# aosokin/os2d

Measured on AMD Instinct MI355X. Metric: query-image-pairs/s (1280-px input, ResNet50, N-class), higher is better.
Workload: dtype fftx3 (as fft; the per-bin complex GEMM on the fp16 MFMA with spectra split into fp16 hi+lo, 3 MFMAs per product, fp32 accumulate)

## Files before the change

os2d_amd/csrc/dft_mfma.h:

```cpp
#pragma once

#ifndef DFT_DEV
#error "the includer defines DFT_DEV, DFT_TID, DFT_BID, DFT_GRID, DFT_LDS, DFT_BARRIER, DFT_MFMA, DFT_SHFL_XOR, DFT_SHFL_XOR_U32, DFT_BALLOT, DFT_FLAG, DFT_FLAG_SET, DFT_RAISE, DFT_UNIFORM"
#endif

#ifndef DFT_HD
#define DFT_HD static inline
#endif
#ifndef DFT_MEMBER
#define DFT_MEMBER inline
#endif
#ifndef DFT_LANDED
#define DFT_LANDED(X)
#endif
#ifndef DFT_FWD_PREFETCH_AFTER
#define DFT_FWD_PREFETCH_AFTER 2
#endif
#ifndef DFT_INV_PREFETCH_AFTER
#define DFT_INV_PREFETCH_AFTER 2
#endif
#ifndef DFT_PIPE_REGA
#define DFT_PIPE_REGA 1
#endif
#ifndef DFT_PIPE_LDS
#define DFT_PIPE_LDS 1
#endif
#ifndef DFT_SCHED_FENCE
#define DFT_SCHED_FENCE()
#endif
#ifndef DFT_STREAM_STORE
#define DFT_STREAM_STORE(P, V) (*(P) = (V))
#endif
#ifndef DFT_STAMP
#define DFT_STAMP(K)
#define DFT_STAMP_BEGIN()
#define DFT_STAMP_END(BASE)
#endif

#include "tile_common.h"

namespace os2d_dft {

typedef float f32x4u __attribute__((ext_vector_type(4), aligned(4)));

constexpr int DFT_THR = 512, DFT_WAVES = 8;
constexpr int DFT_G = 4;
constexpr int DFT_MAXP = 64;
constexpr int DFT_MAXV = 48;
constexpr int DFT_MAXWK = 96;
constexpr int DFT_KREG = 8;

struct DftPlan {
  int H, W;
  int P, Q, V, NBINS;
  int T, TY, TX, TH, TW;
  int oy, ox;
  int LH, LW;
  int RH;
  int Pp;
  int Wk;
  int N1;
  int M2;
  int Mx;
  int N2;
  int MA;
  int MB;
  int KB;
  int NBo;
  int G;
  int eT;
  int fast;
  unsigned inv_cg, inv_t, inv_tx, inv_c4, inv_v, inv_pq, inv_og, inv_kg, inv_pp;
  int lds_const, lds_union, lds_total;
};

DFT_HD int dft_round_up(int x, int m) { return (x + m - 1) / m * m; }
DFT_HD unsigned dft_magic(unsigned d) { return d > 1 ? (unsigned)(((1ull << 32) + d - 1) / d) : 0u; }

DFT_HD int dft_units_fqt(int P, int Q) { return (dft_round_up(Q, 16) / 8) * 2 * dft_round_up(Q + 2, 32); }
DFT_HD int dft_units_fp2(int P, int Q) { return (2 * dft_round_up(P, 8) / 8) * 2 * dft_round_up(2 * P, 32); }
DFT_HD int dft_units_e2(int P, int Q) { return (2 * dft_round_up(P, 8) / 8) * 2 * dft_round_up(2 * P, 32); }
DFT_HD int dft_units_gq(int P, int Q) { return (dft_round_up(Q + 2, 16) / 8) * 2 * dft_round_up(Q, 32); }
DFT_HD size_t dft_matrices_units(int P, int Q) {
  return (size_t)dft_units_fqt(P, Q) + dft_units_fp2(P, Q) + dft_units_e2(P, Q) + dft_units_gq(P, Q);
}

static inline bool dft_plan_transform(int LH, int LW, int RH, int ncols, int minP, int minQ, int G, DftPlan* pl) {
  pl->G = G;
  pl->P = dft_round_up(minP, 4);
  pl->Q = dft_round_up(minQ, 2);
  pl->V = pl->Q / 2 + 1;
  pl->NBINS = dft_round_up(pl->P * pl->V, 8);
  pl->LH = LH;
  pl->LW = LW;
  pl->RH = RH;
  pl->Pp = dft_round_up(pl->P, 8);
  pl->Wk = dft_round_up(LW, 16);
  pl->N1 = dft_round_up(2 * pl->V, 32);
  pl->M2 = dft_round_up(2 * pl->P, 32);
  pl->Mx = dft_round_up(G * pl->Pp, 32);
  pl->N2 = dft_round_up(G * pl->V, 32);
  pl->MA = dft_round_up(2 * RH, 32);
  pl->MB = G * (pl->MA / 2);
  pl->KB = dft_round_up(2 * pl->V, 16);
  pl->NBo = dft_round_up(ncols, 32);
  int e = 0;
  while ((1 << e) < pl->P) ++e;
  pl->eT = e + 1;
  if (pl->P > DFT_MAXP || pl->V > DFT_MAXV || pl->Wk > DFT_MAXWK || LH > pl->P || LW > pl->Q || RH > pl->P) return false;
  const int fqt = (pl->Wk / 8) * 2 * pl->N1 * 16, gq = (pl->KB / 8) * 2 * pl->NBo * 16;
  const int x = (pl->Wk / 8) * 2 * (pl->Mx + 1) * 16, r2 = (2 * pl->Pp / 8) * 2 * (pl->N2 + 1) * 16;
  const int xs = pl->V * (pl->P * 8 * G + 16);
  const int y2 = r2, tt = (pl->KB / 8) * 2 * (pl->MB + 1) * 16;
  int u = x;
  if (r2 > u) u = r2;
  if (xs > u) u = xs;
  if (y2 > u) u = y2;
  if (tt > u) u = tt;
  if (G == 8) {
    const int fp2 = (2 * pl->Pp / 8) * 2 * pl->M2 * 16;
    const int ca = fqt + fp2, cb = gq + fp2;
    pl->lds_const = ca > cb ? ca : cb;
    pl->lds_union = dft_round_up(u, 256);
    pl->lds_total = pl->lds_const + pl->lds_union + 1024;
    const int t1 = (pl->Mx / 32) * (pl->N1 / 32), t2 = (pl->M2 / 32) * (pl->N2 / 32), tA = (pl->MA / 32) * (pl->N2 / 32),
              tB = (pl->MB / 32) * (pl->NBo / 32);
    const int npos = pl->Pp * (pl->Wk / 4), nitem = G * pl->V * (pl->Pp / 8);
    return pl->lds_total <= 160 * 1024 && t1 <= 24 && t2 <= 24 && tA <= 24 && tB <= 24 && npos <= 2 * DFT_THR && nitem <= 3 * DFT_THR;
  }
  pl->lds_const = fqt > gq ? fqt : gq;
  pl->lds_union = dft_round_up(u, 256);
  pl->lds_total = pl->lds_const + pl->lds_union + 1024;
  return pl->lds_total <= 160 * 1024;
}

static inline void dft_set_tiles(DftPlan* pl, int H, int W, int TY, int TX, int TH, int TW) {
  pl->H = H;
  pl->W = W;
  pl->TY = TY;
  pl->TX = TX;
  pl->T = TY * TX;
  pl->TH = TH;
  pl->TW = TW;
  pl->oy = TY > 1 ? 3 : 0;
  pl->ox = TX > 1 ? 3 : 0;
  pl->fast = (pl->T == 1 && (W & 3) == 0) ? 1 : 0;
  pl->inv_t = dft_magic((unsigned)pl->T);
  pl->inv_tx = dft_magic((unsigned)TX);
  pl->inv_c4 = dft_magic((unsigned)(pl->Wk / 4));
  pl->inv_v = dft_magic((unsigned)pl->V);
  pl->inv_pq = dft_magic((unsigned)(pl->P / 4 * pl->G * 2));
  pl->inv_kg = dft_magic((unsigned)(pl->Pp / 8));
  pl->inv_pp = dft_magic((unsigned)pl->Pp);
}

struct DftSize {
  int P, Q;
};
static const DftSize DFT_CANONICAL[6] = {{36, 46}, {44, 54}, {48, 62}, {52, 68}, {56, 70}, {64, 84}};

static inline bool dft_make_plan_policy(int H, int W, int canonical, DftPlan* out, int G = DFT_G) {
  bool found = false;
  long best = 0;
  for (int TY = 1; TY <= 48; ++TY)
    for (int TX = 1; TX <= 48; ++TX) {
      const int TH = (H + TY - 1) / TY, TW = (W + TX - 1) / TX;
      if ((TY > 1 && (TY - 1) * TH >= H) || (TX > 1 && (TX - 1) * TW >= W)) continue;
      const int LH = TY > 1 ? TH + 6 : H, LW = TX > 1 ? TW + 6 : W;
      const int minP = TY > 1 ? TH + 6 : H + 3, minQ = TX > 1 ? TW + 6 : W + 3;
      if (minP > DFT_MAXP || minQ > 2 * (DFT_MAXV - 1)) continue;
      for (int k = 0; k < (canonical ? 6 : 1); ++k) {
        if (canonical && (DFT_CANONICAL[k].P < minP || DFT_CANONICAL[k].Q < minQ)) continue;
        DftPlan c = {};
        if (!dft_plan_transform(LH, LW, TY > 1 ? TH + 3 : H, TX > 1 ? TW + 3 : W, canonical ? DFT_CANONICAL[k].P : minP,
                                canonical ? DFT_CANONICAL[k].Q : minQ, G, &c))
          continue;
        dft_set_tiles(&c, H, W, TY, TX, TH, TW);
        const long cost = (long)c.T * c.NBINS;
        if (!found || cost < best) {
          found = true;
          best = cost;
          *out = c;
        }
      }
    }
  return found;
}

#ifndef OS2D_HOST_EMU
static inline int dft_size_policy() {
  static const int policy = [] {
    const char* e = getenv("OS2D_DFT_SIZES");
    return (e && (e[0] == 'e' || e[0] == '0')) ? 0 : 1;
  }();
  return policy;
}
#else
static inline int dft_size_policy() { return emu_dft_policy; }
#endif
static inline bool dft_make_plan(int H, int W, DftPlan* out) { return dft_make_plan_policy(H, W, dft_size_policy(), out); }
static inline bool dft_plan_g8(const DftPlan& base, DftPlan* out) {
  DftPlan c = {};
  if (!dft_plan_transform(base.LH, base.LW, base.RH, base.TX > 1 ? base.TW + 3 : base.W, base.P, base.Q, 8, &c)) return false;
  dft_set_tiles(&c, base.H, base.W, base.TY, base.TX, base.TH, base.TW);
  *out = c;
  return true;
}

constexpr int DFT_PBLK = 64;
DFT_HD size_t dft_spectra_pair0(int pr, int NBT, int NQ, int cstride, size_t* qstride) {
  const int pb = pr / DFT_PBLK, pl = pr - pb * DFT_PBLK;
  const int nbl = NBT - pb * DFT_PBLK < DFT_PBLK ? NBT - pb * DFT_PBLK : DFT_PBLK;
  *qstride = (size_t)nbl * cstride * 8;
  return ((size_t)pb * DFT_PBLK * NQ + pl) * cstride * 8;
}

DFT_DEV int dft_div(int x, unsigned magic) { return magic ? (int)(((unsigned long long)(unsigned)x * magic) >> 32) : x; }

DFT_DEV void dft_split4(float a, float b, float c, float d, u32x2* hi, u32x2* lo) {
  const f32x4 x = {a, b, c, d};
  const half4 h = __builtin_convertvector(x, half4);
  *hi = __builtin_bit_cast(u32x2, h);
#ifdef DFT_SPLIT_LO_PAIR
  u32x2 l;
  l[0] = DFT_SPLIT_LO_PAIR(a, b, (*hi)[0]);
  l[1] = DFT_SPLIT_LO_PAIR(c, d, (*hi)[1]);
  *lo = l;
#else
  const half4 l = __builtin_convertvector(x - __builtin_convertvector(h, f32x4), half4);
  *lo = __builtin_bit_cast(u32x2, l);
#endif
}

DFT_DEV half8 dft_frag(const u32x4* p) { return __builtin_bit_cast(half8, *p); }

DFT_DEV f32x16 dft_mma3(half8 ah, half8 al, half8 bh, half8 bl, f32x16 acc) {
  acc = DFT_MFMA(ah, bl, acc);
  acc = DFT_MFMA(al, bh, acc);
  acc = DFT_MFMA(ah, bh, acc);
  return acc;
}

template <int NT, int KS>
DFT_DEV void dft_product_rega(f32x16* acc, const half8* ah, const half8* al, int ksn, const u32x4* B, int bstride, int nt0,
                              int ntstep, int l31, int hw) {
  constexpr int KR = KS ? KS : DFT_KREG;
  half8 bh[2][NT], bl[2][NT];
#define DFT_REGA_READ(KSTEP, SET)                                                                                          \
  _Pragma("unroll") for (int j = 0; j < NT; ++j) {                                                                         \
    bh[SET][j] = dft_frag(B + (size_t)((2 * (KSTEP) + hw) * 2 + 0) * bstride + (nt0 + ntstep * j) * 32 + l31);             \
    bl[SET][j] = dft_frag(B + (size_t)((2 * (KSTEP) + hw) * 2 + 1) * bstride + (nt0 + ntstep * j) * 32 + l31);             \
  }
  if (DFT_PIPE_REGA) DFT_REGA_READ(0, 0)
#pragma unroll
  for (int ks = 0; ks < KR; ++ks) {
    if (KS || ks < ksn) {
      if (DFT_PIPE_REGA) {
        if (ks + 1 < KR && (KS || ks + 1 < ksn)) DFT_REGA_READ(ks + 1, (ks + 1) & 1)
        DFT_SCHED_FENCE();
      } else {
        DFT_REGA_READ(ks, ks & 1)
      }
#pragma unroll
      for (int j = 0; j < NT; ++j) acc[j] = dft_mma3(ah[ks], al[ks], bh[ks & 1][j], bl[ks & 1][j], acc[j]);
      if (DFT_PIPE_REGA) DFT_SCHED_FENCE();
    }
  }
#undef DFT_REGA_READ
}

template <int KS>
DFT_DEV void dft_product_rega_any(f32x16* acc, int ntiles, const half8* ah, const half8* al, int ksn, const u32x4* B, int bstride,
                                  int nt0, int ntstep, int l31, int hw) {
  if (ntiles == 3) dft_product_rega<3, KS>(acc, ah, al, ksn, B, bstride, nt0, ntstep, l31, hw);
  else if (ntiles == 2) dft_product_rega<2, KS>(acc, ah, al, ksn, B, bstride, nt0, ntstep, l31, hw);
  else if (ntiles == 1) dft_product_rega<1, KS>(acc, ah, al, ksn, B, bstride, nt0, ntstep, l31, hw);
}

template <int NT, bool SHARE, int NW, int PIPE_MODE>
DFT_DEV void dft_product_lds(f32x16* acc, int ks0, int ks1, const u32x4* A, int astride, const u32x4* B, int bstride, int t0, int mtn,
                             int l31, int hw) {
  constexpr int NA = SHARE ? 1 : NT;
  int tm[NT], tn[NT];
#pragma unroll
  for (int j = 0; j < NT; ++j) {
    const int t = t0 + NW * j;
    tn[j] = t / mtn;
    tm[j] = t - tn[j] * mtn;
  }
  half8 ah[2][NA], al[2][NA], bh[2][NT], bl[2][NT];
#define DFT_LDS_READ(KSTEP, SET)                                                                                           \
  {                                                                                                                        \
    const int kc_ = (KSTEP) < ks1 ? (KSTEP) : ks1 - 1;                                                                     \
    _Pragma("unroll") for (int j = 0; j < NA; ++j) {                                                                       \
      ah[SET][j] = dft_frag(A + (size_t)((2 * kc_ + hw) * 2 + 0) * astride + tm[j] * 32 + l31);                            \
      al[SET][j] = dft_frag(A + (size_t)((2 * kc_ + hw) * 2 + 1) * astride + tm[j] * 32 + l31);                            \
    }                                                                                                                      \
    _Pragma("unroll") for (int j = 0; j < NT; ++j) {                                                                       \
      bh[SET][j] = dft_frag(B + (size_t)((2 * kc_ + hw) * 2 + 0) * bstride + tn[j] * 32 + l31);                            \
      bl[SET][j] = dft_frag(B + (size_t)((2 * kc_ + hw) * 2 + 1) * bstride + tn[j] * 32 + l31);                            \
    }                                                                                                                      \
  }
#define DFT_LDS_MMA(SET)                                                                                                   \
  DFT_SCHED_FENCE();                                                                                                       \
  _Pragma("unroll") for (int j = 0; j < NT; ++j)                                                                           \
    acc[j] = dft_mma3(ah[SET][SHARE ? 0 : j], al[SET][SHARE ? 0 : j], bh[SET][j], bl[SET][j], acc[j]);                    \
  DFT_SCHED_FENCE();
  if (ks0 >= ks1) return;
  constexpr bool PIPE = PIPE_MODE == 2 || (PIPE_MODE == 1 && SHARE);
  if (!PIPE) {
    for (int ks = ks0; ks < ks1; ++ks) {
      DFT_LDS_READ(ks, 0)
      _Pragma("unroll") for (int j = 0; j < NT; ++j)
        acc[j] = dft_mma3(ah[0][SHARE ? 0 : j], al[0][SHARE ? 0 : j], bh[0][j], bl[0][j], acc[j]);
    }
    return;
  }
  DFT_LDS_READ(ks0, 0)
  int ks = ks0;
  for (; ks + 1 < ks1; ks += 2) {
    DFT_LDS_READ(ks + 1, 1)
    DFT_LDS_MMA(0)
    DFT_LDS_READ(ks + 2, 0)
    DFT_LDS_MMA(1)
  }
  if (ks < ks1) {
    DFT_LDS_MMA(0)
  }
#undef DFT_LDS_READ
#undef DFT_LDS_MMA
}

template <int NW, int PIPE_MODE>
DFT_DEV void dft_product_lds_any(f32x16* acc, int ntiles, int ks0, int ks1, const u32x4* A, int astride, const u32x4* B, int bstride,
                                 int t0, int mtn, int l31, int hw) {
  const bool share = mtn == NW;
  if (ntiles == 3) {
    if (share) dft_product_lds<3, true, NW, PIPE_MODE>(acc, ks0, ks1, A, astride, B, bstride, t0, mtn, l31, hw);
    else dft_product_lds<3, false, NW, PIPE_MODE>(acc, ks0, ks1, A, astride, B, bstride, t0, mtn, l31, hw);
  } else if (ntiles == 2) {
    if (share) dft_product_lds<2, true, NW, PIPE_MODE>(acc, ks0, ks1, A, astride, B, bstride, t0, mtn, l31, hw);
    else dft_product_lds<2, false, NW, PIPE_MODE>(acc, ks0, ks1, A, astride, B, bstride, t0, mtn, l31, hw);
  } else if (ntiles == 1) {
    dft_product_lds<1, true, NW, PIPE_MODE>(acc, ks0, ks1, A, astride, B, bstride, t0, mtn, l31, hw);
  }
}

DFT_DEV void dft_matrix_unit(int which, int unit, int P, int Q, const double* twP, const double* twQ, u32x4* out) {
  const int V = Q / 2 + 1, Pp = dft_round_up(P, 8);
  int cols, kidx, hl, col;
  double vals[8];
  if (which == 0) cols = dft_round_up(2 * V, 32);
  else if (which == 1 || which == 2) cols = dft_round_up(2 * P, 32);
  else cols = dft_round_up(Q, 32);
  col = unit % cols;
  hl = (unit / cols) & 1;
  kidx = unit / (2 * cols);
  for (int t = 0; t < 8; ++t) {
    const int k = kidx * 8 + t;
    double x = 0.0;
    if (which == 0) {
      const int v = col >> 1, ri = col & 1;
      if (k < Q && v < V) x = twQ[2 * (int)(((long long)v * k) % Q) + ri] * 16384.0;
    } else if (which == 1) {
      const int ri = k / Pp, h = k - ri * Pp, u = col >> 1, ro = col & 1;
      if (h < P && u < P && ri < 2) {
        const int a = (int)(((long long)u * h) % P);
        const double c = twP[2 * a], s = -twP[2 * a + 1];
        x = (ro == 0 ? (ri == 0 ? c : s) : (ri == 0 ? -s : c)) * 16384.0;
      }
    } else if (which == 2) {
      const int ri = k / Pp, u = k - ri * Pp, h = col >> 1, ro = col & 1;
      if (u < P && h < P && ri < 2) {
        const int a = (int)(((long long)u * h) % P);
        const double c = twP[2 * a], s = -twP[2 * a + 1];
        x = (ro == 0 ? (ri == 0 ? c : -s) : (ri == 0 ? s : c)) * 16384.0;
      }
    } else {
      const int v = k >> 1, ri = k & 1;
      if (v < V && col < Q) {
        const double a = (v == 0 || 2 * v == Q) ? 1.0 : 2.0;
        x = a * twQ[2 * (int)(((long long)v * col) % Q) + ri] * 8192.0;
      }
    }
    vals[t] = x;
  }
  unsigned w[4];
  for (int t = 0; t < 4; ++t) {
    unsigned short b[2];
    for (int e = 0; e < 2; ++e) {
      const double x = vals[2 * t + e];
      const _Float16 h = (_Float16)x;
      const _Float16 r = hl == 0 ? h : (_Float16)(x - (double)h);
      b[e] = __builtin_bit_cast(unsigned short, r);
    }
    w[t] = (unsigned)b[0] | ((unsigned)b[1] << 16);
  }
  u32x4 o;
  o[0] = w[0];
  o[1] = w[1];
  o[2] = w[2];
  o[3] = w[3];
  *out = o;
}

template <bool TILED, bool FAST, int G, int NW, int KS2 = 0>
DFT_DEV void dft_forward_body(const float* corr,
                              const float* invn,
                              float* X,
                              const u32x4* FqT, const u32x4* Fp2, const DftPlan& pl, int C, int Cpad, int NBT, int iters) {
  constexpr int THR = NW * 64;
  constexpr bool ALDS = G == 8;
  unsigned char* smem = DFT_LDS;
  const int tid = DFT_TID, lane = tid & 63, l31 = lane & 31, hw = lane >> 5;
  const int wv = DFT_UNIFORM(tid >> 6);
  const int P = pl.P, V = pl.V, Pp = pl.Pp, Wk = pl.Wk, N1 = pl.N1, Mx = pl.Mx, N2 = pl.N2, LH = pl.LH, LW = pl.LW, W = pl.W, H = pl.H;
  const int MxS = Mx + 1, N2S = N2 + 1;
  const int CG = (C + G - 1) / G, HW = H * W;
  u32x4* ldsF = reinterpret_cast<u32x4*>(smem);
  u32x4* ldsU = reinterpret_cast<u32x4*>(smem + pl.lds_const);
  unsigned char* ldsUb = smem + pl.lds_const;
  const int nF = (Wk / 8) * 2 * N1;
  for (int i = tid; i < nF; i += THR) ldsF[i] = FqT[i];
  u32x4* ldsP = ldsF + nF;
  if (ALDS)
    for (int i = tid; i < (2 * Pp / 8) * 2 * pl.M2; i += THR) ldsP[i] = Fp2[i];

  const int mt1n = Mx / 32, nt1n = N1 / 32, nt2n = N2 / 32, mt2n = pl.M2 / 32;
  const int ks1n = Wk / 16, ks2n = 2 * Pp / 16;
  const int mt2 = wv & 3;
  constexpr int KR2 = KS2 ? KS2 : DFT_KREG;
  half8 fp2h[KR2], fp2l[KR2];
  if (!ALDS) {
#pragma unroll
    for (int ks = 0; ks < KR2; ++ks) {
      const int kc = ks < ks2n ? ks : 0, mc = mt2 < mt2n ? mt2 : 0;
      fp2h[ks] = dft_frag(Fp2 + ((size_t)((2 * kc + hw) * 2 + 0)) * pl.M2 + mc * 32 + l31);
      fp2l[ks] = dft_frag(Fp2 + ((size_t)((2 * kc + hw) * 2 + 1)) * pl.M2 + mc * 32 + l31);
    }
  }
  if (!ALDS) {
#pragma unroll
    for (int ks = 0; ks < KR2; ++ks) {
      DFT_LANDED(fp2h[ks]);
      DFT_LANDED(fp2l[ks]);
    }
  }

  constexpr int NSLOT = ALDS ? 2 : 3 * 512 / THR;
  const int npos = Pp * (Wk / 4);
  f32x4 pc[NSLOT][G], pn[NSLOT];
#define DFT_FWD_ITER(IT)                                                                                     \
  const int pr_ = dft_div((IT), pl.inv_cg), cg_ = (IT)-pr_ * CG;                                             \
  const int nb_ = TILED ? dft_div(pr_, pl.inv_t) : pr_, tile_ = TILED ? pr_ - nb_ * pl.T : 0;               \
  const int ty_ = TILED ? dft_div(tile_, pl.inv_tx) : 0, tx_ = TILED ? tile_ - ty_ * pl.TX : 0;             \
  const int Y0 = TILED ? ty_ * pl.TH - pl.oy : 0, X0 = TILED ? tx_ * pl.TW - pl.ox : 0;                     \
  const int c0_ = cg_ * G;
#define DFT_FWD_POS(TID, S)                                                                                  \
  const int i_ = (TID) + (S)*THR;                                                                        \
  const int r_ = dft_div(i_, pl.inv_c4), c4_ = i_ - r_ * (Wk / 4);                                          \
  const int y_ = Y0 + r_, x_ = X0 + 4 * c4_;
#define DFT_FWD_PREFETCH(IT, TID) DFT_FWD_PREFETCH_SLOTS(IT, TID, 0, NSLOT)
#define DFT_FWD_PREFETCH_SLOTS(IT, TID, S0, S1)                                                              \
  {                                                                                                          \
    DFT_FWD_ITER(IT)                                                                                         \
    _Pragma("unroll") for (int s = (S0); s < (S1); ++s) {                                                    \
      DFT_FWD_POS(TID, s)                                                                                    \
      if (FAST) {                                                                                            \
        const bool ok = i_ < npos && r_ < LH && 4 * c4_ < LW;                                                \
        const int off = ok ? y_ * W + x_ : 0;                                                                \
        pn[s] = *reinterpret_cast<const f32x4*>(invn + (size_t)nb_ * HW + off);                             \
        _Pragma("unroll") for (int g = 0; g < G; ++g) {                                                  \
          const int c = c0_ + g < C ? c0_ + g : C - 1;                                                       \
          pc[s][g] = *reinterpret_cast<const f32x4*>(corr + ((size_t)nb_ * C + c) * HW + off);              \
        }                                                                                                    \
      } else {                                                                                               \
                                                                           \
        const bool rok = i_ < npos && r_ < LH && y_ >= 0 && y_ < H;                                          \
        const int off0 = y_ * W + x_;                                                                        \
        const bool vec = rok && off0 >= 0 && off0 + 3 < HW;                                                  \
        const int offv = vec ? off0 : 0;                                                                     \
        pn[s] = *reinterpret_cast<const f32x4u*>(invn + (size_t)nb_ * HW + offv);                            \
        _Pragma("unroll") for (int g = 0; g < G; ++g) {                                                      \
          const int c = c0_ + g < C ? c0_ + g : C - 1;                                                       \
          pc[s][g] = *reinterpret_cast<const f32x4u*>(corr + ((size_t)nb_ * C + c) * HW + offv);             \
        }                                                                                                    \
        if (rok && !vec) {                                                                                   \
          _Pragma("unroll") for (int e = 0; e < 4; ++e) {                                                    \
            const bool ok = 4 * c4_ + e < LW && x_ + e >= 0 && x_ + e < W;                                   \
            const int off = ok ? y_ * W + x_ + e : 0;                                                        \
            pn[s][e] = invn[(size_t)nb_ * HW + off];                                                         \
            _Pragma("unroll") for (int g = 0; g < G; ++g) {                                                  \
              const int c = c0_ + g < C ? c0_ + g : C - 1;                                                   \
              pc[s][g][e] = corr[((size_t)nb_ * C + c) * HW + off];                                          \
            }                                                                                                \
          }                                                                                                  \
        }                                                                                                    \
      }                                                                                                      \
    }                                                                                                        \
  }
  const int first = (DFT_GRID & 7) == 0 ? (DFT_BID & 7) * (DFT_GRID >> 3) + (DFT_BID >> 3) : DFT_BID;
  if (first < iters) DFT_FWD_PREFETCH(first, tid)
  DFT_BARRIER();

  DFT_STAMP_BEGIN()
  for (int it = first; it < iters; it += DFT_GRID) {
    int tl = tid;
#ifndef OS2D_HOST_EMU
    asm volatile("" : "+v"(tl));
#endif
    const int lane = tl & 63, l31 = lane & 31, hw = lane >> 5;
    DFT_FWD_ITER(it)
    {
#pragma unroll
      for (int s = 0; s < NSLOT; ++s) {
        DFT_FWD_POS(tl, s)
        if (i_ < npos) {
          float nsc[4];
#pragma unroll
          for (int e = 0; e < 4; ++e) {
            const bool ok = FAST ? (r_ < LH && 4 * c4_ < LW) : (r_ < LH && y_ >= 0 && y_ < H && 4 * c4_ + e < LW && x_ + e >= 0 && x_ + e < W);
            nsc[e] = ok ? pn[s][e] * 32768.0f : 0.f;
          }
#pragma unroll
          for (int g = 0; g < G; ++g) {
            u32x2 hi = {0u, 0u}, lo = {0u, 0u};
            if (c0_ + g < C)
              dft_split4(fmaxf(pc[s][g][0], 0.f) * nsc[0], fmaxf(pc[s][g][1], 0.f) * nsc[1], fmaxf(pc[s][g][2], 0.f) * nsc[2],
                         fmaxf(pc[s][g][3], 0.f) * nsc[3], &hi, &lo);
            const int m = g * Pp + r_;
            unsigned char* dst = ldsUb + ((size_t)((c4_ >> 1) * 2) * MxS + m) * 16 + (c4_ & 1) * 8;
            *reinterpret_cast<u32x2*>(dst) = hi;
            *reinterpret_cast<u32x2*>(dst + (size_t)MxS * 16) = lo;
          }
        }
      }
      for (int i = tid; i < (Mx - G * Pp) * (Wk / 8) * 2; i += THR) {
        const int m = G * Pp + i % (Mx - G * Pp), kh = i / (Mx - G * Pp);
        ldsU[(size_t)kh * MxS + m] = u32x4{0u, 0u, 0u, 0u};
      }
    }
    DFT_BARRIER();
    DFT_STAMP(0)

    f32x16 acc[3];
    int tm[3], tn[3];
    int nt1w = 0;
#pragma unroll
    for (int j = 0; j < 3; ++j) {
      const int t = wv + NW * j;
      const bool mine = t < mt1n * nt1n;
      tn[j] = mine ? t / mt1n : 0;
      tm[j] = mine ? t - tn[j] * mt1n : -1;
      nt1w += mine ? 1 : 0;
#pragma unroll
      for (int r = 0; r < 16; ++r) acc[j][r] = 0.f;
    }
    dft_product_lds_any<NW, DFT_PIPE_LDS ? 2 : 0>(acc, nt1w, 0, ks1n, ldsU, MxS, ldsF, N1, wv, mt1n, l31, hw);
    DFT_BARRIER();
    DFT_STAMP(1)

#pragma unroll
    for (int j = 0; j < 3; ++j) {
      if (tm[j] < 0) continue;
      const int n = tn[j] * 32 + l31, v = n >> 1, ri = n & 1;
#pragma unroll
      for (int q = 0; q < 4; ++q) {
        const int mb = tm[j] * 32 + 8 * q;
        const int img = dft_div(mb, pl.inv_pp), h0 = mb - img * Pp + 4 * hw;
        if (v < V && img < G) {
          u32x2 hi, lo;
          const float sc = 1.0f / 2097152.0f;
          dft_split4(acc[j][4 * q] * sc, acc[j][4 * q + 1] * sc, acc[j][4 * q + 2] * sc, acc[j][4 * q + 3] * sc, &hi, &lo);
          const int kg = ri * (Pp / 8) + (h0 >> 3);
          unsigned char* dst = ldsUb + ((size_t)(kg * 2) * N2S + img * V + v) * 16 + (h0 & 4) * 2;
          *reinterpret_cast<u32x2*>(dst) = hi;
          *reinterpret_cast<u32x2*>(dst + (size_t)N2S * 16) = lo;
        }
      }
    }
    DFT_BARRIER();
    DFT_STAMP(2)

    f32x16 xc[3];
    int un[3], um[3];
    int nt2w = 0;
#pragma unroll
    for (int j = 0; j < 3; ++j) {
      const int t = wv + NW * j;
      const int nt = ALDS ? t / mt2n : (wv >> 2) + (NW / 4) * j;
      const bool mine = ALDS ? t < mt2n * nt2n : (nt < nt2n && mt2 < mt2n);
      un[j] = mine ? nt : -1;
      um[j] = ALDS ? t - nt * mt2n : mt2;
      nt2w += mine ? 1 : 0;
#pragma unroll
      for (int r = 0; r < 16; ++r) xc[j][r] = 0.f;
    }
    const int itn = it + DFT_GRID < iters ? it + DFT_GRID : it;
    {
      if (ALDS) {
        dft_product_lds_any<NW, DFT_PIPE_LDS ? 2 : 0>(xc, nt2w, 0, ks2n, ldsP, pl.M2, ldsU, N2S, wv, mt2n, l31, hw);
        DFT_FWD_PREFETCH_SLOTS(itn, tl, 0, NSLOT)
      } else if (DFT_FWD_PREFETCH_AFTER == 1 || (DFT_FWD_PREFETCH_AFTER == 2 && KS2 > 0 && KS2 <= 6)) {
        dft_product_rega_any<KS2>(xc, nt2w, fp2h, fp2l, ks2n, ldsU, N2S, wv >> 2, NW / 4, l31, hw);
        DFT_FWD_PREFETCH_SLOTS(itn, tl, 0, NSLOT)
      } else {
        DFT_FWD_PREFETCH_SLOTS(itn, tl, 0, NSLOT)
        dft_product_rega_any<KS2>(xc, nt2w, fp2h, fp2l, ks2n, ldsU, N2S, wv >> 2, NW / 4, l31, hw);
      }
    }
    DFT_BARRIER();
    DFT_STAMP(3)

    const int XS = P * 8 * G + 16;
#pragma unroll
    for (int j = 0; j < 3; ++j) {
      if (un[j] < 0) continue;
      const int n2 = un[j] * 32 + l31;
      const int img = dft_div(n2, pl.inv_v), v = n2 - img * V;
#pragma unroll
      for (int q = 0; q < 4; ++q) {
        const int u0 = (um[j] * 32 + 8 * q + 4 * hw) >> 1;
        if (img < G && u0 < P) {
          const float sc = 1.0f / 4194304.0f;
          f32x4 o;
          o[0] = xc[j][4 * q] * sc;
          o[1] = xc[j][4 * q + 1] * sc;
          o[2] = xc[j][4 * q + 2] * sc;
          o[3] = xc[j][4 * q + 3] * sc;
          *reinterpret_cast<f32x4*>(ldsUb + (size_t)v * XS + (u0 >> 2) * (G * 32) + img * 32 + (u0 & 3) * 8) = o;
        }
      }
    }
    DFT_BARRIER();
    DFT_STAMP(4)

    {
      const int per_v = (P / 4) * (G * 2), npieces = V * per_v;
      size_t qstride;
      float* dstbase = X + dft_spectra_pair0(pr_, NBT, pl.NBINS / 4, Cpad, &qstride) + (size_t)c0_ * 8;
      for (int i = tl; i < npieces; i += THR) {
        const int v = dft_div(i, pl.inv_pq), rem = i - v * per_v;
        const int uq = rem / (2 * G), jj = rem - uq * (2 * G);
        const f32x4 val = *reinterpret_cast<const f32x4*>(ldsUb + (size_t)v * XS + uq * (G * 32) + jj * 16);
        DFT_STREAM_STORE(reinterpret_cast<f32x4*>(dstbase + (size_t)(v * (P / 4) + uq) * qstride + jj * 4), val);
      }
      const int qpad0 = (P * V) / 4, qpad1 = pl.NBINS / 4;
      for (int i = tl; i < (qpad1 - qpad0) * 2 * G; i += THR)
        *reinterpret_cast<f32x4*>(dstbase + (size_t)(qpad0 + i / (2 * G)) * qstride + (i % (2 * G)) * 4) = f32x4{0.f, 0.f, 0.f, 0.f};
    }
    DFT_BARRIER();
    DFT_STAMP(5)
  }
  DFT_STAMP_END(0)
#undef DFT_FWD_ITER
#undef DFT_FWD_POS
#undef DFT_FWD_PREFETCH
#undef DFT_FWD_PREFETCH_SLOTS
}

template <bool TILED, int KSA = 0, int G = DFT_G>
DFT_DEV void dft_inverse_body(const float* Y,
                              const float* bp,
                              int MTP, unsigned char* out,
                              const u32x4* E2, const u32x4* Gq, const DftPlan& pl, int Cout, int NBT, int PLANE, int Ws,
                              int BASE, int iters, DFT_FLAG bad_flag, int zero_borders) {
  unsigned char* smem = DFT_LDS;
  const int tid = DFT_TID, lane = tid & 63, l31 = lane & 31, hw = lane >> 5;
  const int wv = DFT_UNIFORM(tid >> 6);
  const int P = pl.P, V = pl.V, Pp = pl.Pp, N2 = pl.N2, MB = pl.MB, KB = pl.KB, NBo = pl.NBo, H = pl.H, W = pl.W;
  const int N2S = N2 + 1, MBS = MB + 1;
  const int OG = Cout / G;
  constexpr bool ALDS = G == 8;
  constexpr int LG = G == 8 ? 3 : 2;
  u32x4* ldsG = reinterpret_cast<u32x4*>(smem);
  u32x4* ldsU = reinterpret_cast<u32x4*>(smem + pl.lds_const);
  unsigned char* ldsUb = smem + pl.lds_const;
  float* smaxw = reinterpret_cast<float*>(smem + pl.lds_const + pl.lds_union);
  const int nG = (KB / 8) * 2 * NBo, NQ = dft_round_up(pl.Q, 32);
  for (int i = tid; i < nG; i += DFT_THR) {
    const int kh = i / NBo, n = i - kh * NBo;
    ldsG[i] = Gq[(size_t)kh * NQ + n];
  }
  const int MAfull = dft_round_up(2 * P, 32);
  u32x4* ldsE = ldsG + nG;
  if (ALDS)
    for (int i = tid; i < (2 * Pp / 8) * 2 * MAfull; i += DFT_THR) ldsE[i] = E2[i];

  const int mtAn = pl.MA / 32, ntAn = N2 / 32, ksAn = 2 * Pp / 16;
  const int mtBn = MB / 32, ntBn = NBo / 32, ksBn = KB / 16;
  const int mtA = wv & 3;
  constexpr int KRA = KSA ? KSA : DFT_KREG;
  half8 e2h[KRA], e2l[KRA];
  if (!ALDS) {
#pragma unroll
    for (int ks = 0; ks < KRA; ++ks) {
      const int kc = ks < ksAn ? ks : 0, mc = mtA < mtAn ? mtA : 0;
      e2h[ks] = dft_frag(E2 + ((size_t)((2 * kc + hw) * 2 + 0)) * MAfull + mc * 32 + l31);
      e2l[ks] = dft_frag(E2 + ((size_t)((2 * kc + hw) * 2 + 1)) * MAfull + mc * 32 + l31);
    }
#pragma unroll
    for (int ks = 0; ks < KRA; ++ks) {
      DFT_LANDED(e2h[ks]);
      DFT_LANDED(e2l[ks]);
    }
  }

  constexpr int NITEM = 3;
  const int uoct = Pp / 8, nitem = G * V * uoct;
  f32x4 py[NITEM][4];
#define DFT_INV_PREFETCH(IT, TID) DFT_INV_PREFETCH_ITEMS(IT, TID, 0, NITEM)
#define DFT_INV_PREFETCH_ITEMS(IT, TID, S0, S1)                                             \
  {                                                                                         \
    const int pr_ = dft_div((IT), pl.inv_og), og_ = (IT)-pr_ * OG;                          \
    size_t qstride;                                                                         \
    const float* src_ = Y + dft_spectra_pair0(pr_, NBT, pl.NBINS / 4, Cout, &qstride) + (size_t)og_ * G * 8; \
    _Pragma("unroll") for (int s = (S0); s < (S1); ++s) {                                   \
      const int e_ = (TID) + s * DFT_THR;                                                   \
      const int ec_ = e_ < nitem ? e_ : 0;                                                  \
      const int pimg_ = ec_ & (G - 1), prest_ = ec_ >> LG;                                  \
      const int pv_ = dft_div(prest_, pl.inv_kg), puo_ = prest_ - pv_ * (Pp / 8);           \
      const int q0_ = pv_ * (P / 4) + 2 * puo_;                                             \
      const bool ptwo_ = 8 * puo_ + 4 < P;                                                  \
      const float* p0_ = src_ + (size_t)q0_ * qstride + pimg_ * 8;                          \
      const float* p1_ = src_ + (size_t)(ptwo_ ? q0_ + 1 : q0_) * qstride + pimg_ * 8;      \
      py[s][0] = *reinterpret_cast<const f32x4*>(p0_);                                     \
      py[s][1] = *reinterpret_cast<const f32x4*>(p0_ + 4);                                 \
      py[s][2] = *reinterpret_cast<const f32x4*>(p1_);                                     \
      py[s][3] = *reinterpret_cast<const f32x4*>(p1_ + 4);                                 \
    }                                                                                       \
  }
#define DFT_INV_ITEM(E)                                                                     \
  const int img_ = (E) & (G - 1), rest_ = (E) >> LG;                                        \
  const int v_ = dft_div(rest_, pl.inv_kg), uo_ = rest_ - v_ * uoct;                        \
  const bool two_ = 8 * uo_ + 4 < P;
#define DFT_INV_MAXIMA(TID)                                                                 \
  {                                                                                         \
    float m = 0.f;                                                                          \
    _Pragma("unroll") for (int s = 0; s < NITEM; ++s)                                       \
      if ((TID) + s * DFT_THR < nitem) {                                                    \
        DFT_INV_ITEM((TID) + s * DFT_THR)                                                   \
        (void)img_;                                                                         \
        (void)v_;                                                                           \
        (void)uo_;                                                                          \
        _Pragma("unroll") for (int k = 0; k < 4; ++k)                                       \
          if (k < 2 || two_) {                                                              \
            _Pragma("unroll") for (int e = 0; e < 4; ++e) m = fmaxf(m, fabsf(py[s][k][e])); \
          }                                                                                 \
      }                                                                                     \
    if (G == 4) m = fmaxf(m, DFT_SHFL_XOR(m, 4));                                           \
    m = fmaxf(m, DFT_SHFL_XOR(m, 8));                                                       \
    m = fmaxf(m, DFT_SHFL_XOR(m, 16));                                                      \
    m = fmaxf(m, DFT_SHFL_XOR(m, 32));                                                      \
    if (lane < G) smaxw[wv * G + lane] = m;                                                 \
  }
  bool bad = false;
  const int first = (DFT_GRID & 7) == 0 ? (DFT_BID & 7) * (DFT_GRID >> 3) + (DFT_BID >> 3) : DFT_BID;
  if (first < iters) {
    DFT_INV_PREFETCH(first, tid)
    DFT_INV_MAXIMA(tid)
  }
  DFT_BARRIER();

  DFT_STAMP_BEGIN()
  for (int it = first; it < iters; it += DFT_GRID) {
    int tl = tid;
#ifndef OS2D_HOST_EMU
    asm volatile("" : "+v"(tl));
#endif
    const int lane = tl & 63, l31 = lane & 31, hw = lane >> 5;
    const int pr = dft_div(it, pl.inv_og), og = it - pr * OG;
    const int nb = TILED ? dft_div(pr, pl.inv_t) : pr, tile = TILED ? pr - nb * pl.T : 0;
    const int ty = TILED ? dft_div(tile, pl.inv_tx) : 0, tx = TILED ? tile - ty * pl.TX : 0;
    const int y0 = TILED ? ty * pl.TH : 0, x0 = TILED ? tx * pl.TW : 0, oy = TILED ? pl.oy : 0, ox = TILED ? pl.ox : 0;
    const int TH_ = TILED ? pl.TH : H, TW_ = TILED ? pl.TW : W;
    const int o0 = og * G;

    DFT_STAMP(0)
    float simg = 1.f, cinv[4] = {0.f, 0.f, 0.f, 0.f};
    {
#pragma unroll
      for (int g = 0; g < G; ++g) {
        float m = 0.f;
#pragma unroll
        for (int w = 0; w < DFT_WAVES; ++w) m = fmaxf(m, smaxw[w * G + g]);
        int E = (int)((__builtin_bit_cast(unsigned, m) >> 23) & 0xffu) - 127;
        if (!(m > 0.f) || E < -100) E = -100;
        if (E > 100) E = 100;
        const float s = __builtin_bit_cast(float, (unsigned)(13 - E + 127) << 23);
        const float sinv = __builtin_bit_cast(float, (unsigned)(E - 13 + 127) << 23);
        if (g == (tl & (G - 1))) simg = s;
        const float ci = sinv * __builtin_bit_cast(float, (unsigned)(pl.eT - 13 + 127) << 23) / (float)(P * pl.Q);
        if (G == 4 || (g >> 2) == hw) cinv[g & 3] = ci;
// ... 193 lines not shown
```

os2d_amd/csrc/dft_mfma.hip:

```cpp
#include "tile_common.h"
#include <map>
#include <mutex>
#include <utility>

extern __shared__ __attribute__((aligned(16))) unsigned char os2d_dft_smem[];

#define DFT_DEV __device__ __forceinline__
#define DFT_HD __host__ __device__ static inline
#define DFT_MEMBER __device__ __forceinline__
#define DFT_TID ((int)threadIdx.x)
#define DFT_BID ((int)blockIdx.x)
#define DFT_GRID ((int)gridDim.x)
#define DFT_LDS os2d_dft_smem
#define DFT_BARRIER() asm volatile("s_waitcnt lgkmcnt(0)\n\ts_barrier" ::: "memory")
#define DFT_MFMA(a, b, c) __builtin_amdgcn_mfma_f32_32x32x16_f16(a, b, c, 0, 0, 0)
#define DFT_SHFL_XOR(v, m) __shfl_xor(v, m, 64)
#define DFT_SHFL_XOR_U32(v, m) ((unsigned)__shfl_xor((int)(v), m, 64))
#define DFT_BALLOT(p) __builtin_amdgcn_ballot_w64(p)
#define DFT_UNIFORM(x) __builtin_amdgcn_readfirstlane(x)
#define DFT_SCHED_FENCE() __builtin_amdgcn_sched_barrier(0)
#define DFT_LANDED(X) asm volatile("" : "+v"(X))
#define DFT_SPLIT_LO_PAIR(a, b, hi) os2d_split_lo_pair(a, b, hi)
#define DFT_STREAM_STORE(P, V) os2d_stream_store(P, V)
#define DFT_FLAG Os2dRangeFlag
// ... 12 lines not shown
#define DFT_STAMP_END(BASE)                                                                   \
  if (threadIdx.x == 0) {                                                                     \
    for (int k_ = 0; k_ < 6; ++k_) atomicAdd(&os2d_dft_stamps[(BASE) + k_], st_acc_[k_]);     \
    atomicAdd(&os2d_dft_stamps[(BASE) + 6], st_n_);                                           \
  }
#endif
#include "dft_mfma.h"

namespace {

using namespace os2d_dft;

template <bool TILED, bool FAST, int G, int NW, int KS>
__global__ __launch_bounds__(NW * 64, 8 / NW) void dft_forward_kernel(const float* __restrict__ corr, const float* __restrict__ invn,
                                                                      float* __restrict__ X, const u32x4* __restrict__ FqT,
                                                                      const u32x4* __restrict__ Fp2, DftPlan pl, int C, int Cpad, int NBT,
                                                                      int iters) {
  dft_forward_body<TILED, FAST, G, NW, KS>(corr, invn, X, FqT, Fp2, pl, C, Cpad, NBT, iters);
}

template <bool TILED, int KS, int G>
__global__ __launch_bounds__(DFT_THR, 1) void dft_inverse_kernel(const float* __restrict__ Y, const float* __restrict__ bp, int MTP,
                                                                 unsigned char* __restrict__ out, const u32x4* __restrict__ E2,
                                                                 const u32x4* __restrict__ Gq, DftPlan pl, int Cout, int NBT, int PLANE,
                                                                 int Ws, int BASE, int iters, Os2dRangeFlag status, int zero_borders) {
  dft_inverse_body<TILED, KS, G>(Y, bp, MTP, out, E2, Gq, pl, Cout, NBT, PLANE, Ws, BASE, iters, status, zero_borders);
}

typedef void (*dft_forward_fn)(const float*, const float*, float*, const u32x4*, const u32x4*, DftPlan, int, int, int, int);
typedef void (*dft_inverse_fn)(const float*, const float*, int, unsigned char*, const u32x4*, const u32x4*, DftPlan, int, int, int, int, int,
                               int, Os2dRangeFlag, int);
template <int G, int NW, int KS>
dft_forward_fn dft_forward_variant(const DftPlan& pl) {
  return pl.T > 1 ? dft_forward_kernel<true, false, G, NW, KS> : (pl.fast ? dft_forward_kernel<false, true, G, NW, KS> : dft_forward_kernel<false, false, G, NW, KS>);
}
template <int G, int NW>
dft_forward_fn dft_forward_pick(const DftPlan& pl) {
  if constexpr (G == 8) {
    return dft_forward_variant<G, NW, 0>(pl);
  } else {
    switch (2 * pl.Pp / 16) {
      case 5: return dft_forward_variant<G, NW, 5>(pl);
      case 6: return dft_forward_variant<G, NW, 6>(pl);
      case 7: return dft_forward_variant<G, NW, 7>(pl);
      case 8: return dft_forward_variant<G, NW, 8>(pl);
      default: return dft_forward_variant<G, NW, 0>(pl);
    }
  }
}
template <int KS, int G = DFT_G>
dft_inverse_fn dft_inverse_variant(const DftPlan& pl) {
  return pl.T > 1 ? dft_inverse_kernel<true, KS, G> : dft_inverse_kernel<false, KS, G>;
}
dft_inverse_fn dft_inverse_pick(const DftPlan& pl) {
  if (pl.G == 8) return dft_inverse_variant<0, 8>(pl);
  switch (2 * pl.Pp / 16) {
    case 5: return dft_inverse_variant<5>(pl);
    case 6: return dft_inverse_variant<6>(pl);
    case 7: return dft_inverse_variant<7>(pl);
    case 8: return dft_inverse_variant<8>(pl);
    default: return dft_inverse_variant<0>(pl);
  }
}

__global__ __launch_bounds__(256) void dft_matrices_kernel(const double* __restrict__ twP, const double* __restrict__ twQ, int P, int Q,
                                                           u32x4* __restrict__ out) {
  const int n0 = dft_units_fqt(P, Q), n1 = n0 + dft_units_fp2(P, Q), n2 = n1 + dft_units_e2(P, Q), n3 = n2 + dft_units_gq(P, Q);
  const int i = blockIdx.x * 256 + threadIdx.x;
  if (i >= n3) return;
  const int which = i < n0 ? 0 : i < n1 ? 1 : i < n2 ? 2 : 3;
  const int base = which == 0 ? 0 : which == 1 ? n0 : which == 2 ? n1 : n2;
  dft_matrix_unit(which, i - base, P, Q, twP, twQ, out + i);
}

bool dft_plan_cached(int H, int W, DftPlan* out, bool g8 = true) {
  static const bool g8_enabled = [] {
    const char* e = getenv("OS2D_DFT_G8");
    return !(e && e[0] == '0');
  }();
  struct Entry {
    bool ok, ok8;
    DftPlan pl, pl8;
  };
  static std::mutex mu;
  static std::map<std::pair<int, int>, Entry> cache;
  {
    std::lock_guard<std::mutex> lock(mu);
    auto it = cache.find({H, W});
    if (it != cache.end()) {
      if (it->second.ok) *out = (g8 && g8_enabled && it->second.ok8) ? it->second.pl8 : it->second.pl;
      return it->second.ok;
    }
  }
  Entry e = {};
  e.ok = dft_make_plan(H, W, &e.pl);
  e.ok8 = e.ok && dft_plan_g8(e.pl, &e.pl8);
  if (e.ok) *out = (g8 && g8_enabled && e.ok8) ? e.pl8 : e.pl;
  std::lock_guard<std::mutex> lock(mu);
  if (cache.size() >= 4096) cache.clear();
  cache[{H, W}] = e;
  return e.ok;
}

int dft_grid(int iters, int per_cu = 1) {
  int g = iters < 256 * per_cu ? iters : 256 * per_cu;
  return os2d_round_up(g, 8);
}

}

int os2d_dft_plan(int H, int W, int* P, int* Q, int* nbins, int* tiles) {
  DftPlan pl;
  if (H < 1 || W < 1 || !dft_plan_cached(H, W, &pl)) return 0;
  if (P) *P = pl.P;
  if (Q) *Q = pl.Q;
  if (nbins) *nbins = pl.NBINS;
  if (tiles) {
    tiles[0] = pl.TY;
    tiles[1] = pl.TX;
    tiles[2] = pl.TH;
    tiles[3] = pl.TW;
    tiles[4] = pl.LH;
    tiles[5] = pl.LW;
  }
  return 1;
}

size_t os2d_dft_matrices_size(int P, int Q) { return dft_matrices_units(P, Q) * 16; }

int os2d_launch_dft_matrices(const double* twP64, const double* twQ64, int P, int Q, void* out, hipStream_t stream) {
  if (P < 4 || (P & 3) || P > DFT_MAXP || Q < 2 || (Q & 1) || Q / 2 + 1 > DFT_MAXV) {
    os2d_set_error("dft_matrices: transform %d x %d is outside the kernels' range (P %% 4 == 0, P <= %d, Q even, Q/2 + 1 <= %d)", P, Q,
                   DFT_MAXP, DFT_MAXV);
    return -3;
  }
  const int n = (int)dft_matrices_units(P, Q);
  hipLaunchKernelGGL(dft_matrices_kernel, dim3((n + 255) / 256), dim3(256), 0, stream, twP64, twQ64, P, Q, static_cast<u32x4*>(out));
  return os2d_launched("dft_matrices");
}

int os2d_launch_dft_forward(const float* corr, const float* inv, float* X, const void* matrices, int NB, int C, int Cpad, int H, int W,
                            hipStream_t stream) {
  DftPlan pl;
  if (!dft_plan_cached(H, W, &pl)) {
    os2d_set_error("dft_forward: no transform plan for a %dx%d map", H, W);
    return -3;
  }
  if (pl.G == 8 && Cpad < dft_round_up(C, 8)) dft_plan_cached(H, W, &pl, false);
  const int G = pl.G;
  if (Cpad < dft_round_up(C, G)) {
    os2d_set_error("dft_forward: channel stride %d < %d", Cpad, dft_round_up(C, G));
    return -1;
  }
  const int CG = (C + G - 1) / G, NBT = NB * pl.T, iters = NBT * CG;
  pl.inv_cg = dft_magic((unsigned)CG);
  const u32x4* FqT = static_cast<const u32x4*>(matrices);
  const u32x4* Fp2 = FqT + dft_units_fqt(pl.P, pl.Q);
  auto kern = G == 8 ? dft_forward_pick<8, 8>(pl) : dft_forward_pick<4, 8>(pl);
  if (int rc = os2d_set_dynamic_lds(kern, pl.lds_total, "dft_forward")) return rc;
  hipLaunchKernelGGL(kern, dim3(dft_grid(iters)), dim3(DFT_THR), pl.lds_total, stream, corr, inv, X, FqT, Fp2, pl,
                     C, Cpad, NBT, iters);
  return os2d_launched("dft_forward");
}

int os2d_launch_dft_inverse(const float* Y, const float* bp, int MTP, void* out, const void* matrices, int NB, int Cout, int H, int W,
                            Os2dRangeFlag status, int zero_borders, hipStream_t stream) {
  DftPlan pl;
  if (!dft_plan_cached(H, W, &pl)) {
    os2d_set_error("dft_inverse: no transform plan for a %dx%d map", H, W);
    return -3;
  }
  if (Cout % 8) {
    os2d_set_error("dft_inverse: Cout %d must be a multiple of 8", Cout);
    return -1;
  }
  const int OG = Cout / pl.G, NBT = NB * pl.T, iters = NBT * OG;
  pl.inv_og = dft_magic((unsigned)OG);
  const u32x4* E2 = static_cast<const u32x4*>(matrices) + dft_units_fqt(pl.P, pl.Q) + dft_units_fp2(pl.P, pl.Q);
  const u32x4* Gq = E2 + dft_units_e2(pl.P, pl.Q);
  auto kern = dft_inverse_pick(pl);
  if (int rc = os2d_set_dynamic_lds(kern, pl.lds_total, "dft_inverse")) return rc;
  hipLaunchKernelGGL(kern, dim3(dft_grid(iters)), dim3(DFT_THR), pl.lds_total, stream, Y, bp, MTP, static_cast<unsigned char*>(out), E2, Gq,
                     pl, Cout, NBT, os2d_plane(H, W), os2d_ws(W), os2d_base(W), iters, status, zero_borders);
  return os2d_launched("dft_inverse");
}

extern "C" int os2d_debug_dft_stamps(unsigned long long* out16, int reset) {
#ifdef OS2D_DIAG_DFT_STAMPS
  if (out16 && hipMemcpyFromSymbol(out16, HIP_SYMBOL(os2d_dft_stamps), 16 * sizeof(unsigned long long)) != hipSuccess) return -4;
  if (reset) {
    unsigned long long z[16] = {0};
    if (hipMemcpyToSymbol(HIP_SYMBOL(os2d_dft_stamps), z, sizeof(z)) != hipSuccess) return -4;
  }
  return 0;
#else
  (void)out16, (void)reset;
  os2d_set_error("os2d_debug_dft_stamps: this library was built without -DOS2D_DIAG_DFT_STAMPS");
  return -1;
#endif
}
```

Baseline: 43530.

## Use a radix-2 split for the P=64 row DFT in the forward transform

Rounds a P of 60 up to 64 and, for that size, performs the row DFT as two half-size (32-point) MFMA products on even/odd rows, followed by a twiddle butterfly in the output store loop. This halves the K extent of the second-stage complex GEMM and shrinks the register-held DFT matrix. The cost is a larger transform size, which means more bins and more work in the later stages, plus extra butterfly arithmetic in fp32 and a new reordering of rows. The G=8 path refuses this plan, and the G=4 path errors on non-radix P with Pp=64.

```diff
diff --git a/os2d_amd/csrc/dft_mfma.h b/os2d_amd/csrc/dft_mfma.h
--- a/os2d_amd/csrc/dft_mfma.h
+++ b/os2d_amd/csrc/dft_mfma.h
@@ -78,7 +78,12 @@
 DFT_HD unsigned dft_magic(unsigned d) { return d > 1 ? (unsigned)(((1ull << 32) + d - 1) / d) : 0u; }
 
 DFT_HD int dft_units_fqt(int P, int Q) { return (dft_round_up(Q, 16) / 8) * 2 * dft_round_up(Q + 2, 32); }
-DFT_HD int dft_units_fp2(int P, int Q) { return (2 * dft_round_up(P, 8) / 8) * 2 * dft_round_up(2 * P, 32); }
+constexpr int DFT_R2_P = 64, DFT_R2_MATU = 8 * 2 * 64, DFT_R2_TWU = 16;
+constexpr int DFT_R2_LDS_TW = 512;
+DFT_HD bool dft_radix2(int P) { return P == DFT_R2_P; }
+DFT_HD int dft_units_fp2(int P, int Q) {
+  return dft_radix2(P) ? DFT_R2_MATU + DFT_R2_TWU : (2 * dft_round_up(P, 8) / 8) * 2 * dft_round_up(2 * P, 32);
+}
 DFT_HD int dft_units_e2(int P, int Q) { return (2 * dft_round_up(P, 8) / 8) * 2 * dft_round_up(2 * P, 32); }
 DFT_HD int dft_units_gq(int P, int Q) { return (dft_round_up(Q + 2, 16) / 8) * 2 * dft_round_up(Q, 32); }
 DFT_HD size_t dft_matrices_units(int P, int Q) {
@@ -88,6 +93,7 @@
 static inline bool dft_plan_transform(int LH, int LW, int RH, int ncols, int minP, int minQ, int G, DftPlan* pl) {
   pl->G = G;
   pl->P = dft_round_up(minP, 4);
+  if (pl->P == 60) pl->P = DFT_R2_P;
   pl->Q = dft_round_up(minQ, 2);
   pl->V = pl->Q / 2 + 1;
   pl->NBINS = dft_round_up(pl->P * pl->V, 8);
@@ -118,6 +124,7 @@
   if (y2 > u) u = y2;
   if (tt > u) u = tt;
   if (G == 8) {
+    if (dft_radix2(pl->P)) return false;
     const int fp2 = (2 * pl->Pp / 8) * 2 * pl->M2 * 16;
     const int ca = fqt + fp2, cb = gq + fp2;
     pl->lds_const = ca > cb ? ca : cb;
@@ -347,7 +354,18 @@
 }
 
 DFT_DEV void dft_matrix_unit(int which, int unit, int P, int Q, const double* twP, const double* twQ, u32x4* out) {
-  const int V = Q / 2 + 1, Pp = dft_round_up(P, 8);
+  const int V = Q / 2 + 1;
+  const bool r2 = which == 1 && dft_radix2(P);
+  if (r2 && unit >= DFT_R2_MATU) {
+    const int u = 2 * (unit - DFT_R2_MATU);
+    u32x4 o;
+    for (int t = 0; t < 4; ++t) o[t] = __builtin_bit_cast(unsigned, (float)twP[2 * u + t]);
+    *out = o;
+    return;
+  }
+  const int tws = r2 ? 2 : 1;
+  if (r2) P /= 2;
+  const int Pp = dft_round_up(P, 8);
   int cols, kidx, hl, col;
   double vals[8];
   if (which == 0) cols = dft_round_up(2 * V, 32);
@@ -365,7 +383,7 @@
     } else if (which == 1) {
       const int ri = k / Pp, h = k - ri * Pp, u = col >> 1, ro = col & 1;
       if (h < P && u < P && ri < 2) {
-        const int a = (int)(((long long)u * h) % P);
+        const int a = (int)(((long long)u * h) % P) * tws;
         const double c = twP[2 * a], s = -twP[2 * a + 1];
         x = (ro == 0 ? (ri == 0 ? c : s) : (ri == 0 ? -s : c)) * 16384.0;
       }
@@ -411,6 +429,7 @@
                               const u32x4* FqT, const u32x4* Fp2, const DftPlan& pl, int C, int Cpad, int NBT, int iters) {
   constexpr int THR = NW * 64;
   constexpr bool ALDS = G == 8;
+  constexpr bool R2 = !ALDS && KS2 == 8;
   unsigned char* smem = DFT_LDS;
   const int tid = DFT_TID, lane = tid & 63, l31 = lane & 31, hw = lane >> 5;
   const int wv = DFT_UNIFORM(tid >> 6);
@@ -422,6 +441,8 @@
   unsigned char* ldsUb = smem + pl.lds_const;
   const int nF = (Wk / 8) * 2 * N1;
   for (int i = tid; i < nF; i += THR) ldsF[i] = FqT[i];
+  const unsigned char* ldsTw = smem + pl.lds_const + pl.lds_union + DFT_R2_LDS_TW;
+  if (R2 && tid < DFT_R2_TWU) reinterpret_cast<u32x4*>(smem + pl.lds_const + pl.lds_union + DFT_R2_LDS_TW)[tid] = Fp2[DFT_R2_MATU + tid];
   u32x4* ldsP = ldsF + nF;
   if (ALDS)
     for (int i = tid; i < (2 * Pp / 8) * 2 * pl.M2; i += THR) ldsP[i] = Fp2[i];
@@ -429,9 +450,15 @@
   const int mt1n = Mx / 32, nt1n = N1 / 32, nt2n = N2 / 32, mt2n = pl.M2 / 32;
   const int ks1n = Wk / 16, ks2n = 2 * Pp / 16;
   const int mt2 = wv & 3;
-  constexpr int KR2 = KS2 ? KS2 : DFT_KREG;
+  constexpr int KR2 = R2 ? 4 : KS2 ? KS2 : DFT_KREG;
   half8 fp2h[KR2], fp2l[KR2];
-  if (!ALDS) {
+  if (R2) {
+#pragma unroll
+    for (int ks = 0; ks < KR2; ++ks) {
+      fp2h[ks] = dft_frag(Fp2 + ((size_t)((2 * ks + hw) * 2 + 0)) * 64 + (mt2 & 1) * 32 + l31);
+      fp2l[ks] = dft_frag(Fp2 + ((size_t)((2 * ks + hw) * 2 + 1)) * 64 + (mt2 & 1) * 32 + l31);
+    }
+  } else if (!ALDS) {
 #pragma unroll
     for (int ks = 0; ks < KR2; ++ks) {
       const int kc = ks < ks2n ? ks : 0, mc = mt2 < mt2n ? mt2 : 0;
@@ -528,7 +555,7 @@
             if (c0_ + g < C)
               dft_split4(fmaxf(pc[s][g][0], 0.f) * nsc[0], fmaxf(pc[s][g][1], 0.f) * nsc[1], fmaxf(pc[s][g][2], 0.f) * nsc[2],
                          fmaxf(pc[s][g][3], 0.f) * nsc[3], &hi, &lo);
-            const int m = g * Pp + r_;
+            const int m = g * Pp + (R2 ? (r_ & 1) * 32 + (r_ >> 1) : r_);
             unsigned char* dst = ldsUb + ((size_t)((c4_ >> 1) * 2) * MxS + m) * 16 + (c4_ & 1) * 8;
             *reinterpret_cast<u32x2*>(dst) = hi;
             *reinterpret_cast<u32x2*>(dst + (size_t)MxS * 16) = lo;
@@ -572,7 +599,7 @@
           u32x2 hi, lo;
           const float sc = 1.0f / 2097152.0f;
           dft_split4(acc[j][4 * q] * sc, acc[j][4 * q + 1] * sc, acc[j][4 * q + 2] * sc, acc[j][4 * q + 3] * sc, &hi, &lo);
-          const int kg = ri * (Pp / 8) + (h0 >> 3);
+          const int kg = R2 ? (h0 >> 5) * 8 + ri * 4 + ((h0 & 31) >> 3) : ri * (Pp / 8) + (h0 >> 3);
           unsigned char* dst = ldsUb + ((size_t)(kg * 2) * N2S + img * V + v) * 16 + (h0 & 4) * 2;
           *reinterpret_cast<u32x2*>(dst) = hi;
           *reinterpret_cast<u32x2*>(dst + (size_t)N2S * 16) = lo;
@@ -601,9 +628,12 @@
       if (ALDS) {
         dft_product_lds_any<NW, DFT_PIPE_LDS ? 2 : 0>(xc, nt2w, 0, ks2n, ldsP, pl.M2, ldsU, N2S, wv, mt2n, l31, hw);
         DFT_FWD_PREFETCH_SLOTS(itn, tl, 0, NSLOT)
-      } else if (DFT_FWD_PREFETCH_AFTER == 1 || (DFT_FWD_PREFETCH_AFTER == 2 && KS2 > 0 && KS2 <= 6)) {
+      } else if (!R2 && (DFT_FWD_PREFETCH_AFTER == 1 || (DFT_FWD_PREFETCH_AFTER == 2 && KS2 > 0 && KS2 <= 6))) {
         dft_product_rega_any<KS2>(xc, nt2w, fp2h, fp2l, ks2n, ldsU, N2S, wv >> 2, NW / 4, l31, hw);
         DFT_FWD_PREFETCH_SLOTS(itn, tl, 0, NSLOT)
+      } else if (R2) {
+        DFT_FWD_PREFETCH_SLOTS(itn, tl, 0, NSLOT)
+        dft_product_rega_any<4>(xc, nt2w, fp2h, fp2l, 4, ldsU + (size_t)(mt2 >> 1) * 16 * N2S, N2S, wv >> 2, NW / 4, l31, hw);
       } else {
         DFT_FWD_PREFETCH_SLOTS(itn, tl, 0, NSLOT)
         dft_product_rega_any<KS2>(xc, nt2w, fp2h, fp2l, ks2n, ldsU, N2S, wv >> 2, NW / 4, l31, hw);
@@ -639,6 +669,25 @@
       const int per_v = (P / 4) * (G * 2), npieces = V * per_v;
       size_t qstride;
       float* dstbase = X + dft_spectra_pair0(pr_, NBT, pl.NBINS / 4, Cpad, &qstride) + (size_t)c0_ * 8;
+      if (R2) {
+        constexpr int per_h = (DFT_R2_P / 8) * (G * 2);
+        for (int i = tl; i < V * per_h; i += THR) {
+          const int v = i / per_h, rem = i - v * per_h;
+          const int uq = rem / (2 * G), jj = rem - uq * (2 * G);
+          const unsigned char* src = ldsUb + (size_t)v * XS + uq * (G * 32) + jj * 16;
+          const f32x4 e = *reinterpret_cast<const f32x4*>(src);
+          const f32x4 o = *reinterpret_cast<const f32x4*>(src + (DFT_R2_P / 8) * (G * 32));
+          const f32x4 w = *reinterpret_cast<const f32x4*>(ldsTw + (4 * uq + 2 * (jj & 1)) * 8);
+          f32x4 t;
+          t[0] = w[0] * o[0] - w[1] * o[1];
+          t[1] = w[0] * o[1] + w[1] * o[0];
+          t[2] = w[2] * o[2] - w[3] * o[3];
+          t[3] = w[2] * o[3] + w[3] * o[2];
+          float* dst = dstbase + (size_t)(v * (P / 4) + uq) * qstride + jj * 4;
+          DFT_STREAM_STORE(reinterpret_cast<f32x4*>(dst), e + t);
+          DFT_STREAM_STORE(reinterpret_cast<f32x4*>(dst + (size_t)(DFT_R2_P / 8) * qstride), e - t);
+        }
+      } else
       for (int i = tl; i < npieces; i += THR) {
         const int v = dft_div(i, pl.inv_pq), rem = i - v * per_v;
         const int uq = rem / (2 * G), jj = rem - uq * (2 * G);
diff --git a/os2d_amd/csrc/dft_mfma.hip b/os2d_amd/csrc/dft_mfma.hip
--- a/os2d_amd/csrc/dft_mfma.hip
+++ b/os2d_amd/csrc/dft_mfma.hip
@@ -188,6 +188,10 @@
     os2d_set_error("dft_forward: channel stride %d < %d", Cpad, dft_round_up(C, G));
     return -1;
   }
+  if (G == 4 && pl.Pp == 64 && !dft_radix2(pl.P)) {
+    os2d_set_error("dft_forward: a plan of 8 k-steps with %d rows (the radix-2 kernel takes 64)", pl.P);
+    return -3;
+  }
   const int CG = (C + G - 1) / G, NBT = NB * pl.T, iters = NBT * CG;
   pl.inv_cg = dft_magic((unsigned)CG);
   const u32x4* FqT = static_cast<const u32x4*>(matrices);
```

Result: faster. 44440 (median of 6 runs) (+2.1%).
